# microsoft/GenerativeImage2Text

Hardware: NVIDIA H100
Metric: captions/sec (greedy, max_len=40) GIT_BASE batch64 (higher is better)
Workload: dtype bf16

## Files before the change

generativeimage2text_b200/_lib.py:

```python
import ctypes
import os

HERE = os.path.dirname(os.path.abspath(__file__))
LIB_PATH = os.path.join(HERE, 'libgitb200.so')
ABI_VERSION = 12

c_void_p, c_int, c_int64, c_float, c_char_p = ctypes.c_void_p, ctypes.c_int, ctypes.c_int64, ctypes.c_float, ctypes.c_char_p
c_ll = ctypes.c_longlong


class Config(ctypes.Structure):
    _fields_ = [(n, ctypes.c_int32) for n in (
        'image_size', 'patch', 'enc_width', 'enc_layers', 'enc_heads', 'dec_hidden', 'dec_layers', 'dec_heads',
        'dec_ffn', 'vocab', 'max_positions', 'num_frames_emb', 'sos_id', 'eos_id')]


class Search(ctypes.Structure):
    _fields_ = [('mode', ctypes.c_int32), ('max_steps', ctypes.c_int32), ('beam_size', ctypes.c_int32),
                ('per_node_beam', ctypes.c_int32), ('length_penalty', ctypes.c_float)]


class ImageDesc(ctypes.Structure):
    _fields_ = [('src_offset', ctypes.c_int64), ('src_h', ctypes.c_int32), ('src_w', ctypes.c_int32),
                ('resize_h', ctypes.c_int32), ('resize_w', ctypes.c_int32), ('crop_top', ctypes.c_int32),
                ('crop_left', ctypes.c_int32), ('out_h', ctypes.c_int32), ('out_w', ctypes.c_int32),
                ('dst_offset', ctypes.c_int64)]


# ... 33 lines not shown
    'gitb200_last_decode_ms': (c_int, [c_void_p, ctypes.POINTER(ctypes.c_float), ctypes.POINTER(ctypes.c_int32), ctypes.POINTER(ctypes.c_int32)]),
    'gitb200_set_row_prefixes': (c_int, [c_void_p, c_void_p, c_int, c_int, c_void_p]),
    'gitb200_set_trie': (c_int, [c_void_p, c_void_p, c_void_p, c_void_p, c_int, c_int]),
    'gitb200_set_sampling': (c_int, [c_void_p, c_void_p, c_int, c_int, c_float]),
    'gitb200_set_beam_sampling': (c_int, [c_void_p, c_void_p, c_int, c_int, c_float, c_int, c_float]),
    'gitb200_set_sequences_per_image': (c_int, [c_void_p, c_int]),
    'gitb200_launch_count': (c_int64, [c_void_p]),
    'gitb200_set_option': (c_int, [c_void_p, c_char_p, c_int64]),
    'gitb200_preproc_create': (c_int, [c_int, ctypes.POINTER(c_void_p)]),
    'gitb200_preproc_destroy': (None, [c_void_p]),
    'gitb200_preproc_last_error': (c_char_p, [c_void_p]),
    'gitb200_preproc_launch_count': (c_int64, [c_void_p]),
    'gitb200_preproc_set_option': (c_int, [c_void_p, c_char_p, c_int64]),
    'gitb200_preproc_run': (c_int, [c_void_p, c_void_p, c_int64, c_int, ctypes.POINTER(ImageDesc), c_int,
                                    ctypes.POINTER(c_float), ctypes.POINTER(c_float), c_void_p, c_int64, c_void_p]),
    'gitb200_preproc_coeffs': (c_int, [c_int, c_int, ctypes.POINTER(ctypes.c_int32), c_void_p, c_void_p, c_int]),
    'gitb200_debug_timeline': (c_int, [c_int, c_void_p, c_int]),
    'gitb200_debug_read': (c_ll, [c_void_p, c_char_p, c_void_p, c_ll]),
    'gitb200_op_gemm': (c_int, [c_void_p, c_void_p, c_void_p, c_void_p, c_void_p, c_int, c_int, c_int, c_int, c_int,
                                c_int, c_int, c_int, c_void_p]),
    'gitb200_op_layernorm': (c_int, [c_void_p, c_void_p, c_void_p, c_void_p, c_void_p, c_float, c_void_p, c_void_p,
                                     c_int, c_int, c_void_p]),
    'gitb200_op_gemm_ex': (c_int, [ctypes.POINTER(GemmDesc), ctypes.POINTER(c_int), c_void_p]),
    'gitb200_op_layernorm_ex': (c_int, [c_void_p, c_int, c_ll, c_void_p, c_void_p, c_void_p, c_void_p, c_float, c_void_p,
                                        c_void_p, c_int, c_int, c_int, c_void_p, c_int, c_int, c_int, c_void_p, c_int,
                                        c_void_p]),
    'gitb200_op_lse_combine': (c_int, [c_void_p, c_int, c_int, c_int, c_int, c_void_p, c_void_p, c_float, c_void_p,
                                       c_void_p, c_void_p, c_void_p, c_void_p]),
    'gitb200_op_attention': (c_int, [c_void_p, c_void_p, c_void_p, c_void_p, c_int, c_int, c_int, c_ll, c_ll, c_ll, c_ll,
                                     c_ll, c_ll, c_void_p]),
    'gitb200_op_attention_ex': (c_int, [c_void_p, c_void_p, c_void_p, c_void_p, c_int, c_int, c_int, c_ll, c_ll, c_ll,
                                        c_ll, c_ll, c_ll, ctypes.POINTER(ctypes.c_int32), c_int, c_void_p]),
    'gitb200_score': (c_int, [c_void_p, c_void_p, c_int, c_int, c_void_p, c_void_p, c_void_p, c_int, c_int, c_void_p,
                               c_void_p, c_void_p]),
    'gitb200_op_text_attention': (c_int, [c_void_p, c_void_p, c_void_p, c_void_p, c_void_p, c_void_p, c_int, c_int, c_int,
                                          c_int, ctypes.POINTER(ctypes.c_int32), ctypes.POINTER(ctypes.c_int32), c_int, c_int,
                                          c_void_p]),
    'gitb200_op_decode_attention': (c_int, [c_void_p, c_int, c_void_p, c_void_p, c_void_p, c_void_p, c_void_p, c_void_p,
                                            c_void_p, c_int, c_int, c_int, ctypes.POINTER(ctypes.c_int32), c_int, c_int,
                                            c_int, c_int, c_int, c_void_p]),
    'gitb200_op_beam_sample': (c_int, [c_void_p, c_int, c_int, c_void_p, c_void_p, c_float, c_int, c_float, c_void_p,
                                       c_void_p, c_void_p, c_void_p]),
}

_lib = None

# ... 30 lines not shown
```

generativeimage2text_b200/csrc/decode_mega.cuh:

```cuda
#pragma once
#include "ptx.cuh"
#include "rowops.cuh"

#include <type_traits>

namespace gitb200 {

constexpr int kMegaComputeWarps = 8;
constexpr int kMegaThreads = (kMegaComputeWarps + 1) * 32;
constexpr int kMegaSlots = 12;
constexpr int kMegaSlotBytes = 16384;
constexpr int kMegaTileBytes = 12288;
constexpr int kMegaKvRows = 64;
constexpr int kMegaKvSubRows = 16;
constexpr int kMegaMaxRows = 64;
constexpr int kMegaD = 768, kMegaF = 3072, kMegaH = 12;
constexpr int kMegaAttItems = 6;
constexpr int kMegaOutTiles = kMegaD / 8;
constexpr int kMegaQkvTiles = 3 * kMegaD / 8;
constexpr int kMegaFcTilesPerCta = 3;
constexpr int kMegaFcCtas = kMegaF / 8 / kMegaFcTilesPerCta;
constexpr int kMegaFc2Slices = kMegaF / kMegaD;
constexpr int kMegaMinCtas = kMegaFcCtas;
constexpr int kMegaAttState = 72;
constexpr unsigned int kMegaSpinLimit = 1u << 18;

struct MegaLayer {
  const uint8_t* wqkv;
  const uint8_t* wo;
  const uint8_t* w1;
  const uint8_t* w2;
  const float* bqkv; const float* bo; const float* b1; const float* b2;
  const float* lnag; const float* lnab; const float* lnog; const float* lnob;
  __nv_bfloat16* txt_k;
  __nv_bfloat16* txt_v;
};

struct MegaParams {
  MegaLayer layer[6];
  const uint8_t* lm;
  const float* lm_bias;
  const float* words;
  const float* positions;
  const float* lnemb_g; const float* lnemb_b;
  int M, T_alloc, n_layers;
  float* x;
  float* y;
  float* ypart;
// ... 73 lines not shown
      buf[2 * n] = t; buf[2 * n + 1] = static_cast<unsigned long long>(kid); ++n;
    }
  }
  __device__ __forceinline__ void end() {
    if (buf != nullptr) { mark(700002); if (n < 160u) { buf[2 * n] = globaltimer_ns(); buf[2 * n + 1] = 700003ull; ++n; } }
  }
};
#define MEGA_TL(kid) tlf.mark(kid)
#define MEGA_TL_DEP(a, error) if (((a).lo[5][7] ^ (a).hi[5][7] ^ (a).lo[0][0]) == 0x9E3779B9u) *(error) = kWaitTimelineProbe;
#else
struct MegaTl {
  __device__ __forceinline__ void begin() {}
  __device__ __forceinline__ void mark(int) {}
  __device__ __forceinline__ void end() {}
};
#define MEGA_TL(kid)
#define MEGA_TL_DEP(a, error)
#endif

__device__ __forceinline__ void bulk_load_1d(void* smem_dst, const void* gsrc, uint32_t bytes, uint64_t* bar) {
  asm volatile("cp.async.bulk.shared::cluster.global.mbarrier::complete_tx::bytes [%0], [%1], %2, [%3];"
               ::"r"(smem_u32(smem_dst)), "l"(gsrc), "r"(bytes), "r"(smem_u32(bar)) : "memory");
}
__device__ __forceinline__ bool mbar_wait_bounded(uint64_t* bar, uint32_t parity, const int* error) {
  for (unsigned int i = 0; i < kMegaSpinLimit; ++i) {
    if (mbar_try_wait(bar, parity)) return true;
    if ((i & 1023u) == 1023u && *reinterpret_cast<const volatile int*>(error) != 0) return false;
  }
  return false;
}

struct MegaRing {
  uint8_t* base;
  uint64_t* full;
  uint64_t* empty;
  uint32_t idx;
  int* error;
  volatile uint32_t* issued;
  __device__ __forceinline__ const uint8_t* acquire() {
    const uint32_t slot = idx % kMegaSlots;
    if (!mbar_wait_bounded(&full[slot], (idx / kMegaSlots) & 1, error)) *error = kWaitRingFull;
    return base + slot * kMegaSlotBytes;
  }
  __device__ __forceinline__ const uint8_t* acquire_ahead(uint32_t n) {
    const uint32_t i = idx + n, slot = i % kMegaSlots;
    if (!mbar_wait_bounded(&full[slot], (i / kMegaSlots) & 1, error)) *error = kWaitRingFull;
    return base + slot * kMegaSlotBytes;
  }
  __device__ __forceinline__ void release() {
    __syncwarp();
    if ((threadIdx.x & 31) == 0) mbar_arrive(&empty[idx % kMegaSlots]);
    ++idx;
  }
  __device__ __forceinline__ uint8_t* acquire_at(uint32_t i) {
// ... 643 lines not shown
```

generativeimage2text_b200/csrc/engine_api.inc:

```

extern "C" int gitb200_encode(gitb200_engine* h, const float* images_dev, int batch, int frames, float* feats_out_dev,
                              void* stream) {
  if (!h) return 1;
  const gitb200_engine::NextCall in = take_next_call(h, false);
  ImageBatch ib;
  TRY(image_batch(h, "encode", batch, frames, in.image_hw, &ib));
  if (!images_dev) return fail(h, "encode: null images");
  cudaSetDevice(h->device);
  return encode_impl(h, images_dev, ib, feats_out_dev, static_cast<cudaStream_t>(stream));
}

static int init_src_rows(gitb200_engine* h, cudaStream_t st) {
  const int n = h->cur_rows * h->T_alloc;
  init_src_row_kernel<<<(n + 255) / 256, 256, 0, st>>>(h->src_row[0].as<int>(), h->cur_rows, h->T_alloc);
  CKL(h, "init_src_row_kernel");
  init_src_row_kernel<<<(n + 255) / 256, 256, 0, st>>>(h->src_row[1].as<int>(), h->cur_rows, h->T_alloc);
  CKL(h, "init_src_row_kernel");
  h->cur_src = 0;
  return 0;
}

extern "C" int gitb200_prefill(gitb200_engine* h, int batch, int beam, float* vproj_out_dev, void* stream) {
  if (!h) return 1;
  cudaSetDevice(h->device);
// ... 158 lines not shown
  CKL(h, "greedy_select_kernel");
  return 0;
}

static int work_stream(gitb200_engine* h, cudaStream_t user, cudaStream_t* out) {
  if (user != nullptr && user != cudaStreamLegacy && user != cudaStreamPerThread) {
    *out = user;
    return 0;
  }
  if (h->own_stream == nullptr) {
    CK(cudaStreamCreateWithFlags(&h->own_stream, cudaStreamNonBlocking));
    CK(cudaEventCreateWithFlags(&h->own_event, cudaEventDisableTiming));
  }
  CK(cudaEventRecord(h->own_event, user));
  CK(cudaStreamWaitEvent(h->own_stream, h->own_event, 0));
  *out = h->own_stream;
  return 0;
}

static int generate_finish(gitb200_engine* h, int32_t* out_len_host) {
  if (!h->pending) return fail(h, "generate_finish: no generate call in flight");
  CK(cudaStreamSynchronize(h->pend_stream));
  h->pending = false;
  if (h->host_state[3].error != 0)
    return fail(h, "decode_mega_kernel: a bounded wait gave up (code %d: %s)", h->host_state[3].error,
                mega_wait_error_name(h->host_state[3].error));
  if (h->host_state[3].bad_draw != 0) {
    const int at = 0x7fffffff - h->host_state[3].bad_draw;
    return fail(h, "beam sampling: step %d, row %d has fewer than two tokens of non-zero probability to draw "
                "(torch.multinomial raises on it)", at / h->pend_rows, at % h->pend_rows);
  }
  if (out_len_host) {
    if (h->pend_beam) {
      *out_len_host = h->pend_max_steps;
    } else {
      *out_len_host = h->host_state[3].empty_caption ? -1 : h->host_state[3].final_len;
    }
  }
  return 0;
}

static int grow_text_cache(gitb200_engine* h, int new_T, SearchCtx* c, cudaStream_t st) {
  const int D = h->D, R = h->cur_rows, nl = h->cfg.dec_layers, old_T = h->T_alloc;
  if (new_T <= old_T) return 0;
  DevBuf nkv, nsrc[2];
  const size_t eb = h->kvb();
// ... 561 lines not shown
                d.row_offset, static_cast<long long>(d.batch_stride));
  GemmCall c;
  c.A = static_cast<const bf16*>(d.a); c.lda = d.lda; c.B = static_cast<const bf16*>(d.b); c.ldb = d.ldb;
  c.bn = d.bn;
  GemmParams& p = c.p;
  p.M = d.M; p.N = d.N; p.K = d.K; p.k_splits = d.k_splits;
  p.transposed = d.transposed ? 1 : 0; p.partial = d.k_splits > 1 ? 1 : 0; p.split_stride = d.split_stride;
  p.act = d.act; p.out_bf16 = d.out_bf16 ? 1 : 0; p.split3 = d.split3 ? 1 : 0;
  p.bias = d.bias; p.resid = d.resid; p.ld_resid = d.ld_resid;
  for (int s = 0; s < 3; ++s) p.out[s] = d.out[s];
  p.ldo = d.ldo; p.seg_n = d.seg_n;
  p.rows_per_batch = d.rows_per_batch; p.batch_stride = d.batch_stride; p.row_offset = d.rows_per_batch > 0 ? d.row_offset : 0;
  p.lse_target = d.lse_target; p.skip = d.skip;
  if (k_splits_out) *k_splits_out = effective_k_splits(d.K, d.k_splits);
  return launch_gemm(h, c, st);
}

extern "C" int gitb200_op_gemm_ex(const gitb200_gemm_desc* desc, int* k_splits_out, void* stream) {
  gitb200_engine* h = op_engine();
  if (!h) return fail(nullptr, "op_gemm_ex: no CUDA device");
  const int rc = desc ? op_gemm_ex_impl(h, *desc, k_splits_out, static_cast<cudaStream_t>(stream))
                      : fail(h, "op_gemm_ex: null descriptor");
  if (rc != 0) g_create_error = h->err;
  return rc;
}

static int op_layernorm_ex_impl(gitb200_engine* h, LnParams p, int D, int pre, cudaStream_t st) {
  if (!p.x || !p.gamma || !p.beta) return fail(h, "op_layernorm_ex: null input");
  if (p.rows < 1) return fail(h, "op_layernorm_ex: rows %d < 1", p.rows);
  if (p.n_partials < 1) return fail(h, "op_layernorm_ex: n_partials %d < 1", p.n_partials);
  if (p.n_partials > 1 && p.partial_stride < static_cast<long long>(p.rows) * D)
    return fail(h, "op_layernorm_ex: partial_stride smaller than one partial buffer");
  if (p.split3 && !p.out_bf16) return fail(h, "op_layernorm_ex: split3 is a bf16 output format");
  if (p.remap_F < 0 || (p.remap_F > 0 && (p.remap_B < 1 || p.remap_L < 1 || p.rows != p.remap_B * p.remap_F * p.remap_L)))
    return fail(h, "op_layernorm_ex: %d rows are not B=%d x F=%d x L=%d", p.rows, p.remap_B, p.remap_F, p.remap_L);
  if (p.temb && p.remap_F == 0) return fail(h, "op_layernorm_ex: a temporal embedding needs the frame remap");
  if (pre && D != 768) return fail(h, "op_layernorm_ex: the PRE instantiation exists for D = 768 only");
  return launch_ln(h, p, D, st, pre != 0);
}

extern "C" int gitb200_op_layernorm_ex(const float* x_dev, int n_partials, long long partial_stride, const float* bias_dev,
                                       const float* resid_dev, const float* gamma_dev, const float* beta_dev, float eps,
                                       float* out_f32_dev, void* out_bf16_dev, int rows, int D, int split3,
                                       const float* temb_dev, int remap_B, int remap_F, int remap_L,
                                       const int32_t* skip_flag_dev, int pre, void* stream) {
  gitb200_engine* h = op_engine();
// ... 292 lines not shown
```

generativeimage2text_b200/csrc/gemm.cuh:

```cuda
#pragma once
#include "ptx.cuh"

namespace gitb200 {

struct GemmParams {
  int M, N, K;
  int k_splits;
  int transposed;
  int partial;
  long long split_stride;
  int act;
  int out_bf16;
  const float* bias;
  const float* resid;
  long long ld_resid;
  void* out[3];
  long long ldo;
  long long batch_stride;
  int seg_n;
  int rows_per_batch;
  int row_offset;
  const int* skip;
  unsigned long long* dbg;
  int split3;
  int pdl;
  ChainSync chain;
  const int* lse_target;
};

constexpr int EPI_TRANSPOSED = 1, EPI_BF16 = 2, EPI_RESID = 4, EPI_PARTIAL = 8, EPI_ACT_SHIFT = 4, EPI_SPLIT3 = 64;
constexpr int EPI_LSE = 128;
constexpr int epi_code(bool transposed, bool bf16, bool resid, bool partial, int act) {
  return (transposed ? EPI_TRANSPOSED : 0) | (bf16 ? EPI_BF16 : 0) | (resid ? EPI_RESID : 0) | (partial ? EPI_PARTIAL : 0) |
         (act << EPI_ACT_SHIFT);
}

template <int ACT>
__device__ __forceinline__ float act_ct(float x) {
  return apply_act(x, ACT);
}

template <int BN>
struct GemmCfg {
  static constexpr int BM = 128;
  static constexpr int BK = 64;
  static constexpr int A_BYTES = BM * BK * 2;
  static constexpr int B_BYTES = BN * BK * 2;
  static constexpr int STAGE_BYTES = A_BYTES + B_BYTES;
  static constexpr int MMA_WGS = 2;
  static constexpr int THREADS = 128 * (1 + MMA_WGS);
// ... 176 lines not shown
  for (int it = 0; it < 8; ++it) {
    const int rr = it * 4 + rsub;
    const float4 v = *reinterpret_cast<const float4*>(stg + rr * 128 + ((c4 ^ (rr & 7)) << 4));
    const float x[4] = {v.x + b[0], v.y + b[1], v.z + b[2], v.w + b[3]};
    float cm = -INFINITY;
#pragma unroll
    for (int e = 0; e < 4; ++e) if (ok[e]) cm = fmaxf(cm, x[e]);
    const float nm = fmaxf(m[it], cm);
    if (nm == -INFINITY) continue;
    float acc = (m[it] == -INFINITY) ? 0.f : se[it] * __expf(m[it] - nm);
#pragma unroll
    for (int e = 0; e < 4; ++e) {
      if (ok[e]) {
        acc += __expf(x[e] - nm);
        sx[it] += x[e];
        if (tgt[it] == col0 + e) xt[it] = x[e];
      }
    }
    se[it] = acc;
    m[it] = nm;
  }
}

template <int BN, int EPI>
__global__ void __launch_bounds__(GemmCfg<BN>::THREADS, 1)
gemm_bf16_wgmma(const __grid_constant__ CUtensorMap tmA, const __grid_constant__ CUtensorMap tmB,
                const GemmParams p) {
  using C = GemmCfg<BN>;
  constexpr bool kTransposed = (EPI & EPI_TRANSPOSED) != 0;
  constexpr bool kLse = (EPI & EPI_LSE) != 0;
  static_assert(!kLse || EPI == EPI_LSE, "the statistics epilogue takes no other option");
  if (p.pdl) griddep_launch_early();
  if (p.pdl) tl_mark(100000 + 1000 + static_cast<int>(gridDim.x));
  if ((!p.pdl || p.chain.counters != nullptr) && p.skip != nullptr && *p.skip != 0) return;
  extern __shared__ __align__(1024) uint8_t smem_raw[];
  uint8_t* smem = smem_raw + ((1024u - (smem_u32(smem_raw) & 1023u)) & 1023u);
  uint8_t* sA = smem;
  uint8_t* sB = smem + C::STAGES * C::A_BYTES;
  uint8_t* sStage = smem + C::STAGES * C::STAGE_BYTES;
  uint64_t* full = reinterpret_cast<uint64_t*>(sStage + C::STAGING_BYTES);
  uint64_t* empty = full + C::STAGES;

  const int wg = threadIdx.x >> 7;
  const int warp = (threadIdx.x >> 5) & 3;
  const int lane = threadIdx.x & 31;

  if (threadIdx.x == 0) {
    tma_prefetch_desc(&tmA);
    tma_prefetch_desc(&tmB);
    for (int s = 0; s < C::STAGES; ++s) {
      mbar_init(&full[s], 1);
      mbar_init(&empty[s], C::MMA_WGS);
    }
    mbar_fence_init();
  }
  __syncthreads();

  const int m_tiles = (p.M + C::BM - 1) / C::BM;
  const int n_tiles = (p.N + BN - 1) / BN;
  const int kb_total = (p.K + C::BK - 1) / C::BK;
  const int kb_per = (kb_total + p.k_splits - 1) / p.k_splits;
  const int mn_tiles = m_tiles * n_tiles;
  const int num_tiles = mn_tiles * p.k_splits;

  const bool chained = p.chain.counters != nullptr;
  int npre = 0;
  if (kTransposed && p.pdl && static_cast<int>(blockIdx.x) < num_tiles) {
    const int split = static_cast<int>(blockIdx.x) / mn_tiles;
    const int kb0 = split * kb_per;
    npre = min(C::STAGES, min(kb_total, kb0 + kb_per) - kb0);
    if (threadIdx.x == 0) {
      const int m_blk = (static_cast<int>(blockIdx.x) - split * mn_tiles) / n_tiles;
      for (int i = 0; i < npre; ++i) {
        mbar_arrive_expect_tx(&full[i], C::STAGE_BYTES);
        tma_load_2d(sA + i * C::A_BYTES, &tmA, &full[i], (kb0 + i) * C::BK, m_blk * C::BM);
      }
    }
  }
  if (chained) chain_wait(p.chain);
  else if (p.pdl) griddep_wait();
  if (p.pdl) tl_mark(1000 + static_cast<int>(gridDim.x));

  if (wg == 0) {
    setmaxnreg_dec<C::PRODUCER_REGS>();
    if (threadIdx.x == 0) {
      int stage = 0;
      uint32_t phase = 0;
      for (int tile = blockIdx.x; tile < num_tiles; tile += gridDim.x) {
        const int split = tile / mn_tiles;
        const int rem = tile - split * mn_tiles;
        const int m_blk = rem / n_tiles;
        const int n_blk = rem - m_blk * n_tiles;
        const int kb0 = split * kb_per;
        const int kb1 = min(kb_total, kb0 + kb_per);
        for (int kb = kb0; kb < kb1; ++kb) {
          if (npre > 0) {
            --npre;
            tma_load_2d(sB + stage * C::B_BYTES, &tmB, &full[stage], kb * C::BK, n_blk * BN);
          } else {
            mbar_wait(&empty[stage], phase ^ 1);
            mbar_arrive_expect_tx(&full[stage], C::STAGE_BYTES);
            tma_load_2d(sA + stage * C::A_BYTES, &tmA, &full[stage], kb * C::BK, m_blk * C::BM);
            tma_load_2d(sB + stage * C::B_BYTES, &tmB, &full[stage], kb * C::BK, n_blk * BN);
          }
          if (++stage == C::STAGES) {
            stage = 0;
            phase ^= 1;
          }
        }
      }
    }
  } else {
    setmaxnreg_inc<C::MMA_REGS>();
    const int mw = wg - 1;
    const bool store_ok = !(p.pdl && !chained && p.skip != nullptr && *p.skip != 0);
    uint8_t* stg_wg = sStage + mw * C::WG_STAGING_BYTES;
    uint8_t* stg = stg_wg + warp * (32 * 128);
    const int rsub = lane >> 3;
    float acc[BN / 2];
    int stage = 0;
    uint32_t phase = 0;
    for (int tile = blockIdx.x; tile < num_tiles; tile += gridDim.x) {
      const int split = tile / mn_tiles;
      const int rem = tile - split * mn_tiles;
      const int m_blk = rem / n_tiles;
      const int n_blk = rem - m_blk * n_tiles;
      const int kb0 = split * kb_per;
      const int kb1 = min(kb_total, kb0 + kb_per);
      int prev = -1;
      for (int kb = kb0; kb < kb1; ++kb) {
        mbar_wait(&full[stage], phase);
        if (p.pdl && tile == static_cast<int>(blockIdx.x) && kb == kb0 && threadIdx.x == 128) tl_mark_one(300000 + 1000 + static_cast<int>(gridDim.x));
        const uint32_t a_base = smem_u32(sA + stage * C::A_BYTES + mw * (64 * 128));
        const uint32_t b_base = smem_u32(sB + stage * C::B_BYTES);
        wgmma_fence();
#pragma unroll
        for (int k = 0; k < C::BK / 16; ++k)
          Wgmma<BN>::mma(acc, wgmma_desc_sw128(a_base + k * 32), wgmma_desc_sw128(b_base + k * 32), (kb > kb0 || k > 0) ? 1u : 0u);
        wgmma_commit();
        if (prev >= 0) {
          wgmma_wait<1>();
          if ((threadIdx.x & 127) == 0) mbar_arrive(&empty[prev]);
        }
        prev = stage;
        if (++stage == C::STAGES) {
          stage = 0;
          phase ^= 1;
        }
      }
      wgmma_wait<0>();
      if ((threadIdx.x & 127) == 0) mbar_arrive(&empty[prev]);
      if (p.pdl && tile == static_cast<int>(blockIdx.x) && threadIdx.x == 128) tl_mark_one(400000 + 1000 + static_cast<int>(gridDim.x));

      const int row0 = m_blk * C::BM + mw * 64 + (warp & 1) * 32;
      long long ooff[8];
      uint32_t okmask = 0;
      if (!kTransposed && !kLse) okmask = epi_row_offsets(p, row0, rsub, store_ok, ooff);
      float lm[8], lse_s[8], lsx[8], lxt[8];
      int ltg[8];
      if constexpr (kLse) {
#pragma unroll
        for (int it = 0; it < 8; ++it) {
          const int row = row0 + it * 4 + rsub;
          ltg[it] = row < p.M ? p.lse_target[row] : -1;
          lm[it] = -INFINITY; lse_s[it] = 0.f; lsx[it] = 0.f; lxt[it] = 0.f;
        }
      }
#pragma unroll
      for (int cc = 0; cc < BN / 64; ++cc) {
        if (n_blk * BN + cc * 64 >= p.N) break;
#pragma unroll
        for (int j8 = 0; j8 < 8; ++j8) {
#pragma unroll
          for (int hh = 0; hh < 2; ++hh) {
// ... 25 lines not shown
#pragma unroll
        for (int it = 0; it < 8; ++it) {
#pragma unroll
          for (int o = 1; o < 8; o <<= 1) {
            const float m_o = __shfl_xor_sync(0xffffffffu, lm[it], o);
            const float s_o = __shfl_xor_sync(0xffffffffu, lse_s[it], o);
            const float nm = fmaxf(lm[it], m_o);
            const float sa = (lm[it] == -INFINITY) ? 0.f : lse_s[it] * __expf(lm[it] - nm);
            const float sb = (m_o == -INFINITY) ? 0.f : s_o * __expf(m_o - nm);
            lse_s[it] = sa + sb;
            lm[it] = nm;
            lsx[it] += __shfl_xor_sync(0xffffffffu, lsx[it], o);
            lxt[it] += __shfl_xor_sync(0xffffffffu, lxt[it], o);
          }
          const int row = row0 + it * 4 + rsub;
          if ((lane & 7) == 0 && row < p.M)
            reinterpret_cast<float4*>(p.out[0])[static_cast<long long>(row) * p.ldo + 2 * n_blk + (warp >> 1)] =
                make_float4(lm[it], lse_s[it], lsx[it], lxt[it]);
        }
      }
    }
  }

  __syncthreads();
  if (p.pdl) tl_mark(200000 + 1000 + static_cast<int>(gridDim.x));
  if (chained && threadIdx.x == 0) chain_signal_thread0(p.chain);
}

}
```

generativeimage2text_b200/csrc/gitb200.cu:

```cuda
#include <cuda.h>
#include <cuda_bf16.h>
#include <cuda_runtime.h>

#include <algorithm>
#include <atomic>
#include <cmath>
#include <cstdarg>
#include <cstdio>
#include <cstring>
#include <map>
#include <mutex>
#include <set>
#include <string>
#include <utility>
#include <vector>

#include "../../include/gitb200.h"
#include "attention.cuh"
#include "constrained.cuh"
#include "decode_mega.cuh"
#include "gemm.cuh"
#include "preproc.cuh"
#include "ptx.cuh"
#include "rowops.cuh"
#include "search.cuh"

using namespace gitb200;
typedef __nv_bfloat16 bf16;

#define GITB200_ABI_VERSION 12

static thread_local std::string g_create_error;

struct DevBuf {
  static inline std::atomic<unsigned long long> moves{0};
  void* p = nullptr;
  size_t cap = 0;
  bool owned = true;
  cudaError_t ensure(size_t bytes) {
    if (bytes <= cap) return cudaSuccess;
    if (!owned) return cudaErrorInvalidValue;
    if (p) cudaFree(p);
    p = nullptr;
    cap = 0;
    ++moves;
    cudaError_t e = cudaMalloc(&p, bytes);
    if (e == cudaSuccess) cap = bytes;
    return e;
  }
  void release() {
    if (p) ++moves;
    if (p && owned) cudaFree(p);
    p = nullptr;
// ... 88 lines not shown
  DevBuf img_kv, txt_kv, src_row[2];
  size_t txt_kv_eb = 0;
  DevBuf xd_t, hd_t, qkv_t, ctx_t, t_t, u_t, logits;
  DevBuf y_t, qb_t, mega_bar;
  DevBuf state, next_token, logprob_sum, tokens_i64, stage_img, stage_tok, stage_lp, prefix_dev;
  DevBuf beam_ws;
  BeamState beam_s{};
  int beam_B = 0, beam_max_steps = 0;
  int beam_cand = 0;
  DevBuf sc_kv, sc_tgt, sc_part, sc_loss, sc_valid, sc_index;
  DevBuf sel_ws;
  DevBuf chain;
  DecAttnGeom attn_geom{};
  int cur_B = 0, cur_frames = 0, cur_M = 0, cur_beam = 1, T_alloc = 0, cur_rows = 0, cur_src = 0;
  int cur_seqs = 1;

  EncodeTiledFn encode_tiled = nullptr;
  std::map<TmapKey, CUtensorMap> tmaps;

  struct StepGraph { cudaGraphExec_t exec = nullptr; int64_t launches = 0; unsigned long long last_use = 0; };
  std::map<std::string, StepGraph> step_graphs;
  unsigned long long step_graph_clock = 0;
  int last_gemm_grid = 0;
  cudaStream_t own_stream = nullptr;
  cudaEvent_t own_event = nullptr;
  StepState* host_state = nullptr;
  bool pending = false;
  int pend_max_steps = 0;
  int pend_rows = 0;
  bool pend_beam = false;
  cudaStream_t pend_stream = nullptr;
  cudaEvent_t chunk_ev[2] = {nullptr, nullptr};
  cudaEvent_t dec_ev[2] = {nullptr, nullptr};
  int dec_steps = 0;
  bool dec_mega = false;
  DevBuf trie_begin, trie_token, trie_child, trie_cursor;
  int trie_nodes = 0;
  struct NextCall {
    std::vector<int> image_hw;
    const long long* prefix_tok = nullptr;
    const int32_t* prefix_lens = nullptr;
    int prefix_rows = 0, prefix_stride = 0;
    const float* uniforms = nullptr;
    int sample_steps = 0, sample_rows = 0;
    float temperature = 1.0f;
    const float* beam_uniforms = nullptr;
// ... 99 lines not shown

static int set_dyn_smem(gitb200_engine* h, const void* kernel, size_t smem) {
  static std::mutex mu;
  static std::map<std::pair<const void*, int>, size_t> done;
  std::lock_guard<std::mutex> lock(mu);
  size_t& have = done[{kernel, h->device}];
  if (have < smem) {
    CK(cudaFuncSetAttribute(kernel, cudaFuncAttributeMaxDynamicSharedMemorySize, static_cast<int>(smem)));
    have = smem;
  }
  return 0;
}

struct GemmCall {
  const bf16* A = nullptr;
  long long lda = 0;
  const bf16* B = nullptr;
  long long ldb = 0;
  GemmParams p{};
  int bn = 0;
};

template <int BN, int EPI>
static int launch_gemm_inst(gitb200_engine* h, const GemmCall& c, cudaStream_t st) {
  using C = GemmCfg<BN>;
  TRY(set_dyn_smem(h, reinterpret_cast<const void*>(gemm_bf16_wgmma<BN, EPI>), C::SMEM_BYTES));
  CUtensorMap ta, tb;
  TRY(get_tmap(h, c.A, c.p.M, c.p.K, c.lda, 128, &ta));
  TRY(get_tmap(h, c.B, c.p.N, c.p.K, c.ldb, BN, &tb));
  const int m_tiles = (c.p.M + 127) / 128;
  const int n_tiles = (c.p.N + BN - 1) / BN;
  const int tiles = m_tiles * n_tiles * c.p.k_splits;
  const int grid = tiles < h->num_sms ? tiles : h->num_sms;
  h->last_gemm_grid = grid;
  CK(launch_k(c.p.pdl != 0, gemm_bf16_wgmma<BN, EPI>, dim3(grid), dim3(C::THREADS), C::SMEM_BYTES, st, ta, tb, c.p));
  CKL(h, "gemm_bf16_wgmma");
  return 0;
}

template <int BN>
static int launch_gemm_bn(gitb200_engine* h, const GemmCall& c, cudaStream_t st) {
  const GemmParams& p = c.p;
  if constexpr (BN == 256) {
    if (p.lse_target != nullptr) return launch_gemm_inst<BN, EPI_LSE>(h, c, st);
  }
  if (p.lse_target != nullptr) return fail(h, "gemm: the LM-head statistics epilogue runs with 256-column tiles only");
  const int code = epi_code(p.transposed != 0, p.out_bf16 != 0, p.resid != nullptr, p.partial != 0, p.act) | (p.split3 ? EPI_SPLIT3 : 0);
  if constexpr (BN == 256) {
    switch (code) {
      case epi_code(false, true, false, false, ACT_QUICKGELU_EXACT) | EPI_SPLIT3: return launch_gemm_inst<BN, epi_code(false, true, false, false, ACT_QUICKGELU_EXACT) | EPI_SPLIT3>(h, c, st);
      case epi_code(false, true, false, false, ACT_GELU_ERF) | EPI_SPLIT3: return launch_gemm_inst<BN, epi_code(false, true, false, false, ACT_GELU_ERF) | EPI_SPLIT3>(h, c, st);
      default: break;
    }
  }
// ... 359 lines not shown
  logprob_sum[r] = 0.f;
}
__global__ void advance_prefix_kernel(StepState* st, long long* next_token, const long long* prefix, int idx, int rows,
                                      unsigned int* chain) {
  const int r = blockIdx.x * blockDim.x + threadIdx.x;
  if (r < rows) next_token[r] = prefix[idx];
  if (r == 0) st->pos = st->pos + 1;
  if (r < 64) chain[r] = 0;
}

extern "C" int gitb200_abi_version(void) { return GITB200_ABI_VERSION; }

extern "C" const char* gitb200_last_error(const gitb200_engine* h) { return h ? h->err.c_str() : g_create_error.c_str(); }

extern "C" int64_t gitb200_launch_count(const gitb200_engine* h) { return h ? h->launches : 0; }

extern "C" int gitb200_set_option(gitb200_engine* h, const char* name, int64_t value) {
  if (!h || !name) return 1;
  drop_step_graphs(h);
  if (strcmp(name, "use_graph") == 0) { h->use_graph = value != 0; return 0; }
  if (strcmp(name, "use_pdl") == 0) { h->use_pdl = value != 0; return 0; }
  if (strcmp(name, "use_mega") == 0) { h->use_mega = value != 0; return 0; }
  if (strcmp(name, "debug_layers") == 0) { h->debug_layers = static_cast<int>(value); return 0; }
  if (strcmp(name, "parity") == 0) {
    if (h->weights_from != nullptr) return fail(h, "parity: this engine borrows its weights; switch the owning engine");
    if (h->parity != (value != 0)) { h->parity = value != 0; h->finalized = false; h->seen.clear(); h->tmaps.clear(); }
    return 0;
  }
  return fail(h, "unknown option %s", name);
}

static int check_image_size(gitb200_engine* h, const char* what, int b, int height, int width) {
  const int p = h->cfg.patch;
  const long long tokens = static_cast<long long>(height / p) * (width / p) + 1;
  if (b < 0) {
    if (height < p || width < p) return fail(h, "%s: %dx%d is smaller than one %dx%d patch", what, height, width, p, p);
    if (tokens > 16384) return fail(h, "%s: %dx%d gives %lld tokens per image (limit 16384)", what, height, width, tokens);
    return 0;
  }
  if (height < p || width < p) return fail(h, "%s: image %d is %dx%d, smaller than one %dx%d patch", what, b, height, width, p, p);
  if (tokens > 16384) return fail(h, "%s: image %d (%dx%d) gives %lld tokens (limit 16384)", what, b, height, width, tokens);
  return 0;
}

extern "C" int gitb200_set_input_size(gitb200_engine* h, int height, int width) {
  if (!h) return 1;
// ... 654 lines not shown
```

generativeimage2text_b200/csrc/ptx.cuh:

```cuda
#pragma once
#include <cuda.h>
#include <cuda_bf16.h>
#include <cuda_runtime.h>
#include <stdint.h>

namespace gitb200 {

__device__ __forceinline__ uint32_t smem_u32(const void* p) {
  return static_cast<uint32_t>(__cvta_generic_to_shared(p));
}
__device__ __forceinline__ int lane_id() { return threadIdx.x & 31; }
__device__ __forceinline__ unsigned long long globaltimer_ns() {
  unsigned long long t;
  asm volatile("mov.u64 %0, %%globaltimer;" : "=l"(t));
  return t;
}

#ifdef GITB200_TIMELINE
__device__ unsigned long long* g_tl_buf = nullptr;
__device__ unsigned int g_tl_count = 0;
constexpr unsigned int kTimelineMax = 8192;
__device__ __forceinline__ void tl_mark_one(int kid) {
  if (g_tl_buf != nullptr && blockIdx.x == 0 && blockIdx.y == 0 && blockIdx.z == 0) {
    const unsigned int i = atomicAdd(&g_tl_count, 1u);
// ... 68 lines not shown
  asm volatile("mbarrier.arrive.expect_tx.shared::cta.b64 _, [%0], %1;" ::"r"(smem_u32(bar)), "r"(bytes)
               : "memory");
}
__device__ __forceinline__ void mbar_arrive(uint64_t* bar) {
  asm volatile("mbarrier.arrive.shared::cta.b64 _, [%0];" ::"r"(smem_u32(bar)) : "memory");
}
__device__ __forceinline__ bool mbar_try_wait(uint64_t* bar, uint32_t parity) {
  uint32_t ok;
  asm volatile(
      "{\n"
      ".reg .pred p;\n"
      "mbarrier.try_wait.parity.shared::cta.b64 p, [%1], %2;\n"
      "selp.u32 %0, 1, 0, p;\n"
      "}\n"
      : "=r"(ok)
      : "r"(smem_u32(bar)), "r"(parity)
      : "memory");
  return ok != 0;
}
__device__ __forceinline__ void mbar_wait(uint64_t* bar, uint32_t parity) {
  while (!mbar_try_wait(bar, parity)) {
  }
}

__device__ __forceinline__ void tma_prefetch_desc(const CUtensorMap* m) {
  asm volatile("prefetch.tensormap [%0];" ::"l"(reinterpret_cast<uint64_t>(m)) : "memory");
}
__device__ __forceinline__ void tma_load_2d(void* smem_dst, const CUtensorMap* m, uint64_t* bar, int c_inner,
                                            int c_outer) {
  asm volatile(
      "cp.async.bulk.tensor.2d.shared::cluster.global.mbarrier::complete_tx::bytes [%0], [%1, {%3, %4}], [%2];"
      ::"r"(smem_u32(smem_dst)), "l"(reinterpret_cast<uint64_t>(m)), "r"(smem_u32(bar)), "r"(c_inner),
      "r"(c_outer)
      : "memory");
}

__device__ __forceinline__ void wgmma_fence() { asm volatile("wgmma.fence.sync.aligned;" ::: "memory"); }
__device__ __forceinline__ void wgmma_commit() { asm volatile("wgmma.commit_group.sync.aligned;" ::: "memory"); }
template <int N>
__device__ __forceinline__ void wgmma_wait() {
  asm volatile("wgmma.wait_group.sync.aligned %0;" ::"n"(N) : "memory");
}
template <int R>
__device__ __forceinline__ void setmaxnreg_dec() { asm volatile("setmaxnreg.dec.sync.aligned.u32 %0;" ::"n"(R)); }
template <int R>
__device__ __forceinline__ void setmaxnreg_inc() { asm volatile("setmaxnreg.inc.sync.aligned.u32 %0;" ::"n"(R)); }

__device__ __forceinline__ uint64_t wgmma_desc_sw128(uint32_t smem_addr) {
  uint64_t d = 0;
  d |= static_cast<uint64_t>((smem_addr & 0x3FFFF) >> 4);
  d |= static_cast<uint64_t>(1) << 16;
  d |= static_cast<uint64_t>(1024 >> 4) << 32;
  d |= static_cast<uint64_t>(1) << 62;
  return d;
}

// ... 159 lines not shown
```

include/gitb200.h:

```cpp
#ifndef GITB200_H_
#define GITB200_H_

#include <stdint.h>

#ifdef __cplusplus
extern "C" {
#endif

typedef struct gitb200_engine gitb200_engine;

typedef struct gitb200_config {
  int32_t image_size;
  int32_t patch;
  int32_t enc_width;
  int32_t enc_layers;
  int32_t enc_heads;
  int32_t dec_hidden;
  int32_t dec_layers;
  int32_t dec_heads;
  int32_t dec_ffn;
  int32_t vocab;
  int32_t max_positions;
  int32_t num_frames_emb;
  int32_t sos_id;
// ... 71 lines not shown
int64_t gitb200_launch_count(const gitb200_engine* h);
int gitb200_set_option(gitb200_engine* h, const char* name, int64_t value);

int gitb200_op_gemm(const void* a_dev, const void* w_dev, const float* bias_dev, const float* resid_dev,
                    void* out_dev, int M, int N, int K, int act, int out_bf16, int transposed, int k_splits,
                    int bn, void* stream);
int gitb200_op_layernorm(const float* x_dev, const float* bias_dev, const float* resid_dev, const float* gamma_dev,
                         const float* beta_dev, float eps, float* out_f32_dev, void* out_bf16_dev, int rows, int D,
                         void* stream);
typedef struct gitb200_gemm_desc {
  const void* a;
  const void* b;
  const float* bias;
  const float* resid;
  void* out[3];
  const int32_t* lse_target;
  const int32_t* skip;
  int64_t lda, ldb, ld_resid, ldo, batch_stride, split_stride;
  int32_t M, N, K;
  int32_t act, out_bf16, split3, transposed, k_splits, bn;
  int32_t seg_n, rows_per_batch, row_offset;
} gitb200_gemm_desc;
int gitb200_op_gemm_ex(const gitb200_gemm_desc* desc, int* k_splits_out, void* stream);
int gitb200_op_layernorm_ex(const float* x_dev, int n_partials, long long partial_stride, const float* bias_dev,
                            const float* resid_dev, const float* gamma_dev, const float* beta_dev, float eps,
                            float* out_f32_dev, void* out_bf16_dev, int rows, int D, int split3, const float* temb_dev,
                            int remap_B, int remap_F, int remap_L, const int32_t* skip_flag_dev, int pre, void* stream);
int gitb200_op_lse_combine(const void* parts_dev, int n_parts, int rows, int T, int V, const int32_t* targets_dev,
                           const int64_t* need_predict_dev, float eps, float* logprob_dev, float* row_loss_dev,
                           int32_t* row_valid_dev, float* loss_dev, void* stream);
int gitb200_op_attention(const void* q_dev, const void* k_dev, const void* v_dev, void* out_dev, int B, int S, int H,
                         long long q_row_stride, long long kv_row_stride, long long q_batch_stride,
                         long long kv_batch_stride, long long out_row_stride, long long out_batch_stride,
                         void* stream);
int gitb200_op_attention_ex(const void* q_dev, const void* k_dev, const void* v_dev, void* out_dev, int B, int S, int H,
                            long long q_row_stride, long long kv_row_stride, long long q_batch_stride,
                            long long kv_batch_stride, long long out_row_stride, long long out_batch_stride,
                            const int32_t* seq_lens_host, int fp32, void* stream);
int gitb200_op_decode_attention(const float* qkv_dev, int n_partials, const float* bqkv_dev, const void* img_k_dev,
                                const void* img_v_dev, void* txt_k_dev, void* txt_v_dev, const int32_t* src_row_dev,
                                void* ctx_dev, int B, int beam, int M, const int32_t* img_lens_host, int T_alloc, int pos,
                                int D, int fp32, int grid, void* stream);

int gitb200_op_beam_sample(const float* logits_dev, int rows, int V, const float* beam_scores_dev, const float* uniforms_dev,
                           float temperature, int top_k, float top_p, float* cand_val_out_dev, int32_t* cand_idx_out_dev,
                           int32_t* kept_out_dev, void* stream);
// ... 33 lines not shown
```

Before: 3013.

## Add 2-CTA cluster GEMM variant with TMA multicast of shared B tiles

Adds a paired form of the wgmma GEMM where two CTAs in a cluster compute adjacent M tiles and each loads half of the shared B tile, multicasting it to both CTAs. Empty-slot barriers are released across the cluster. A heuristic picks the paired form when the estimated bytes loaded per round drop, and only for non-PDL, non-chained plain-epilogue GEMMs. The aim is to cut global and L2 traffic for the weight operand, at the cost of cluster synchronisation, bounded spin waits that report errors, and an extra device-to-host error check at generate_finish.

```diff
diff --git a/generativeimage2text_b200/_lib.py b/generativeimage2text_b200/_lib.py
--- a/generativeimage2text_b200/_lib.py
+++ b/generativeimage2text_b200/_lib.py
@@ -3,7 +3,7 @@
 
 HERE = os.path.dirname(os.path.abspath(__file__))
 LIB_PATH = os.path.join(HERE, 'libgitb200.so')
-ABI_VERSION = 12
+ABI_VERSION = 13
 
 c_void_p, c_int, c_int64, c_float, c_char_p = ctypes.c_void_p, ctypes.c_int, ctypes.c_int64, ctypes.c_float, ctypes.c_char_p
 c_ll = ctypes.c_longlong
@@ -83,6 +83,7 @@
     'gitb200_op_layernorm': (c_int, [c_void_p, c_void_p, c_void_p, c_void_p, c_void_p, c_float, c_void_p, c_void_p,
                                      c_int, c_int, c_void_p]),
     'gitb200_op_gemm_ex': (c_int, [ctypes.POINTER(GemmDesc), ctypes.POINTER(c_int), c_void_p]),
+    'gitb200_op_gemm_pair': (c_int, [c_int]),
     'gitb200_op_layernorm_ex': (c_int, [c_void_p, c_int, c_ll, c_void_p, c_void_p, c_void_p, c_void_p, c_float, c_void_p,
                                         c_void_p, c_int, c_int, c_int, c_void_p, c_int, c_int, c_int, c_void_p, c_int,
                                         c_void_p]),
diff --git a/generativeimage2text_b200/csrc/decode_mega.cuh b/generativeimage2text_b200/csrc/decode_mega.cuh
--- a/generativeimage2text_b200/csrc/decode_mega.cuh
+++ b/generativeimage2text_b200/csrc/decode_mega.cuh
@@ -23,7 +23,7 @@
 constexpr int kMegaFc2Slices = kMegaF / kMegaD;
 constexpr int kMegaMinCtas = kMegaFcCtas;
 constexpr int kMegaAttState = 72;
-constexpr unsigned int kMegaSpinLimit = 1u << 18;
+constexpr unsigned int kMegaSpinLimit = kSpinLimit;
 
 struct MegaLayer {
   const uint8_t* wqkv;
@@ -143,14 +143,6 @@
   asm volatile("cp.async.bulk.shared::cluster.global.mbarrier::complete_tx::bytes [%0], [%1], %2, [%3];"
                ::"r"(smem_u32(smem_dst)), "l"(gsrc), "r"(bytes), "r"(smem_u32(bar)) : "memory");
 }
-__device__ __forceinline__ bool mbar_wait_bounded(uint64_t* bar, uint32_t parity, const int* error) {
-  for (unsigned int i = 0; i < kMegaSpinLimit; ++i) {
-    if (mbar_try_wait(bar, parity)) return true;
-    if ((i & 1023u) == 1023u && *reinterpret_cast<const volatile int*>(error) != 0) return false;
-  }
-  return false;
-}
-
 struct MegaRing {
   uint8_t* base;
   uint64_t* full;
diff --git a/generativeimage2text_b200/csrc/engine_api.inc b/generativeimage2text_b200/csrc/engine_api.inc
--- a/generativeimage2text_b200/csrc/engine_api.inc
+++ b/generativeimage2text_b200/csrc/engine_api.inc
@@ -204,6 +204,7 @@
   if (!h->pending) return fail(h, "generate_finish: no generate call in flight");
   CK(cudaStreamSynchronize(h->pend_stream));
   h->pending = false;
+  TRY(check_gemm_waits(h, h->pend_stream));
   if (h->host_state[3].error != 0)
     return fail(h, "decode_mega_kernel: a bounded wait gave up (code %d: %s)", h->host_state[3].error,
                 mega_wait_error_name(h->host_state[3].error));
@@ -811,6 +812,18 @@
   const int rc = desc ? op_gemm_ex_impl(h, *desc, k_splits_out, static_cast<cudaStream_t>(stream))
                       : fail(h, "op_gemm_ex: null descriptor");
   if (rc != 0) g_create_error = h->err;
+  return rc;
+}
+
+extern "C" int gitb200_op_gemm_pair(int mode) {
+  gitb200_engine* h = op_engine();
+  if (!h) return fail(nullptr, "op_gemm_pair: no CUDA device");
+  int rc = 0;
+  if (mode < -1 || mode > 1) rc = fail(h, "op_gemm_pair: mode %d is not -1, 0 or 1", mode);
+  else if (cudaDeviceSynchronize() != cudaSuccess) rc = fail(h, "op_gemm_pair: device synchronise failed");
+  else rc = check_gemm_waits(h, nullptr);
+  if (rc == 0) h->gemm_pair = mode;
+  else g_create_error = h->err;
   return rc;
 }
 
diff --git a/generativeimage2text_b200/csrc/gemm.cuh b/generativeimage2text_b200/csrc/gemm.cuh
--- a/generativeimage2text_b200/csrc/gemm.cuh
+++ b/generativeimage2text_b200/csrc/gemm.cuh
@@ -26,6 +26,12 @@
   int pdl;
   ChainSync chain;
   const int* lse_target;
+  int* error;
+};
+
+enum GemmWaitError : int {
+  kGemmWaitFull = 1,
+  kGemmWaitEmpty = 2,
 };
 
 constexpr int EPI_TRANSPOSED = 1, EPI_BF16 = 2, EPI_RESID = 4, EPI_PARTIAL = 8, EPI_ACT_SHIFT = 4, EPI_SPLIT3 = 64;
@@ -248,7 +254,11 @@
   }
 }
 
-template <int BN, int EPI>
+__host__ __device__ constexpr bool gemm_pairable(int epi) {
+  return (epi & (EPI_TRANSPOSED | EPI_PARTIAL | EPI_SPLIT3 | EPI_LSE)) == 0;
+}
+
+template <int BN, int EPI, bool kPair = false>
 __global__ void __launch_bounds__(GemmCfg<BN>::THREADS, 1)
 gemm_bf16_wgmma(const __grid_constant__ CUtensorMap tmA, const __grid_constant__ CUtensorMap tmB,
                 const GemmParams p) {
@@ -256,6 +266,8 @@
   constexpr bool kTransposed = (EPI & EPI_TRANSPOSED) != 0;
   constexpr bool kLse = (EPI & EPI_LSE) != 0;
   static_assert(!kLse || EPI == EPI_LSE, "the statistics epilogue takes no other option");
+  static_assert(!kPair || gemm_pairable(EPI), "the paired form runs the plain normal shape only");
+  constexpr int kHalfB = C::B_BYTES / 2;
   if (p.pdl) griddep_launch_early();
   if (p.pdl) tl_mark(100000 + 1000 + static_cast<int>(gridDim.x));
   if ((!p.pdl || p.chain.counters != nullptr) && p.skip != nullptr && *p.skip != 0) return;
@@ -276,18 +288,23 @@
     tma_prefetch_desc(&tmB);
     for (int s = 0; s < C::STAGES; ++s) {
       mbar_init(&full[s], 1);
-      mbar_init(&empty[s], C::MMA_WGS);
+      mbar_init(&empty[s], C::MMA_WGS * (kPair ? 2 : 1));
     }
     mbar_fence_init();
   }
   __syncthreads();
+  if constexpr (kPair) cluster_sync();
+  const uint32_t rank = kPair ? cluster_ctarank() : 0u;
 
   const int m_tiles = (p.M + C::BM - 1) / C::BM;
   const int n_tiles = (p.N + BN - 1) / BN;
   const int kb_total = (p.K + C::BK - 1) / C::BK;
   const int kb_per = (kb_total + p.k_splits - 1) / p.k_splits;
-  const int mn_tiles = m_tiles * n_tiles;
+  const int m_units = kPair ? (m_tiles + 1) / 2 : m_tiles;
+  const int mn_tiles = m_units * n_tiles;
   const int num_tiles = mn_tiles * p.k_splits;
+  const int first_tile = kPair ? static_cast<int>(blockIdx.x) / 2 : static_cast<int>(blockIdx.x);
+  const int tile_step = kPair ? static_cast<int>(gridDim.x) / 2 : static_cast<int>(gridDim.x);
 
   const bool chained = p.chain.counters != nullptr;
   int npre = 0;
@@ -312,15 +329,22 @@
     if (threadIdx.x == 0) {
       int stage = 0;
       uint32_t phase = 0;
-      for (int tile = blockIdx.x; tile < num_tiles; tile += gridDim.x) {
+      for (int tile = first_tile; tile < num_tiles; tile += tile_step) {
         const int split = tile / mn_tiles;
         const int rem = tile - split * mn_tiles;
-        const int m_blk = rem / n_tiles;
-        const int n_blk = rem - m_blk * n_tiles;
+        const int m_unit = rem / n_tiles;
+        const int n_blk = rem - m_unit * n_tiles;
+        const int m_blk = kPair ? 2 * m_unit + static_cast<int>(rank) : m_unit;
         const int kb0 = split * kb_per;
         const int kb1 = min(kb_total, kb0 + kb_per);
         for (int kb = kb0; kb < kb1; ++kb) {
-          if (npre > 0) {
+          if constexpr (kPair) {
+            if (!mbar_wait_bounded(&empty[stage], phase ^ 1, p.error)) *p.error = kGemmWaitEmpty;
+            mbar_arrive_expect_tx(&full[stage], C::STAGE_BYTES);
+            tma_load_2d(sA + stage * C::A_BYTES, &tmA, &full[stage], kb * C::BK, m_blk * C::BM);
+            tma_load_2d_multicast(sB + stage * C::B_BYTES + rank * kHalfB, &tmB, &full[stage], kb * C::BK,
+                                  n_blk * BN + static_cast<int>(rank) * (BN / 2), 0x3);
+          } else if (npre > 0) {
             --npre;
             tma_load_2d(sB + stage * C::B_BYTES, &tmB, &full[stage], kb * C::BK, n_blk * BN);
           } else {
@@ -346,16 +370,31 @@
     float acc[BN / 2];
     int stage = 0;
     uint32_t phase = 0;
-    for (int tile = blockIdx.x; tile < num_tiles; tile += gridDim.x) {
+    auto release = [&](int slot) {
+      if ((threadIdx.x & 127) == 0) {
+        if constexpr (kPair) {
+          mbar_arrive_cluster(&empty[slot], 0);
+          mbar_arrive_cluster(&empty[slot], 1);
+        } else {
+          mbar_arrive(&empty[slot]);
+        }
+      }
+    };
+    for (int tile = first_tile; tile < num_tiles; tile += tile_step) {
       const int split = tile / mn_tiles;
       const int rem = tile - split * mn_tiles;
-      const int m_blk = rem / n_tiles;
-      const int n_blk = rem - m_blk * n_tiles;
+      const int m_unit = rem / n_tiles;
+      const int n_blk = rem - m_unit * n_tiles;
+      const int m_blk = kPair ? 2 * m_unit + static_cast<int>(rank) : m_unit;
       const int kb0 = split * kb_per;
       const int kb1 = min(kb_total, kb0 + kb_per);
       int prev = -1;
       for (int kb = kb0; kb < kb1; ++kb) {
-        mbar_wait(&full[stage], phase);
+        if constexpr (kPair) {
+          if (!mbar_wait_bounded(&full[stage], phase, p.error)) *p.error = kGemmWaitFull;
+        } else {
+          mbar_wait(&full[stage], phase);
+        }
         if (p.pdl && tile == static_cast<int>(blockIdx.x) && kb == kb0 && threadIdx.x == 128) tl_mark_one(300000 + 1000 + static_cast<int>(gridDim.x));
         const uint32_t a_base = smem_u32(sA + stage * C::A_BYTES + mw * (64 * 128));
         const uint32_t b_base = smem_u32(sB + stage * C::B_BYTES);
@@ -366,7 +405,7 @@
         wgmma_commit();
         if (prev >= 0) {
           wgmma_wait<1>();
-          if ((threadIdx.x & 127) == 0) mbar_arrive(&empty[prev]);
+          release(prev);
         }
         prev = stage;
         if (++stage == C::STAGES) {
@@ -375,7 +414,7 @@
         }
       }
       wgmma_wait<0>();
-      if ((threadIdx.x & 127) == 0) mbar_arrive(&empty[prev]);
+      release(prev);
       if (p.pdl && tile == static_cast<int>(blockIdx.x) && threadIdx.x == 128) tl_mark_one(400000 + 1000 + static_cast<int>(gridDim.x));
 
       const int row0 = m_blk * C::BM + mw * 64 + (warp & 1) * 32;
@@ -447,7 +486,8 @@
     }
   }
 
-  __syncthreads();
+  if constexpr (kPair) cluster_sync();
+  else __syncthreads();
   if (p.pdl) tl_mark(200000 + 1000 + static_cast<int>(gridDim.x));
   if (chained && threadIdx.x == 0) chain_signal_thread0(p.chain);
 }
diff --git a/generativeimage2text_b200/csrc/gitb200.cu b/generativeimage2text_b200/csrc/gitb200.cu
--- a/generativeimage2text_b200/csrc/gitb200.cu
+++ b/generativeimage2text_b200/csrc/gitb200.cu
@@ -28,7 +28,7 @@
 using namespace gitb200;
 typedef __nv_bfloat16 bf16;
 
-#define GITB200_ABI_VERSION 12
+#define GITB200_ABI_VERSION 13
 
 static thread_local std::string g_create_error;
 
@@ -163,6 +163,8 @@
   std::map<std::string, StepGraph> step_graphs;
   unsigned long long step_graph_clock = 0;
   int last_gemm_grid = 0;
+  int gemm_pair = -1;
+  DevBuf gemm_err;
   cudaStream_t own_stream = nullptr;
   cudaEvent_t own_event = nullptr;
   StepState* host_state = nullptr;
@@ -308,14 +310,100 @@
 };
 
 template <int BN, int EPI>
+static int pair_clusters(gitb200_engine* h, int* out) {
+  using C = GemmCfg<BN>;
+  static std::mutex mu;
+  static std::map<int, int> done;
+  const auto kern = gemm_bf16_wgmma<BN, EPI, true>;
+  TRY(set_dyn_smem(h, reinterpret_cast<const void*>(kern), C::SMEM_BYTES));
+  std::lock_guard<std::mutex> lock(mu);
+  auto it = done.find(h->device);
+  if (it == done.end()) {
+    cudaLaunchConfig_t cfg{};
+    cfg.gridDim = dim3(2 * h->num_sms);
+    cfg.blockDim = dim3(C::THREADS);
+    cfg.dynamicSmemBytes = C::SMEM_BYTES;
+    cudaLaunchAttribute attr[1];
+    attr[0].id = cudaLaunchAttributeClusterDimension;
+    attr[0].val.clusterDim.x = 2; attr[0].val.clusterDim.y = 1; attr[0].val.clusterDim.z = 1;
+    cfg.attrs = attr;
+    cfg.numAttrs = 1;
+    int n = 0;
+    CK(cudaOccupancyMaxActiveClusters(&n, kern, &cfg));
+    it = done.emplace(h->device, n).first;
+  }
+  *out = it->second;
+  return 0;
+}
+
+static bool gemm_pair_wins(int m_tiles, int n_tiles, int a_bytes, int b_bytes, int sms, int clusters) {
+  const long long rounds = (static_cast<long long>(m_tiles) * n_tiles + sms - 1) / sms;
+  const long long pair_rounds = (static_cast<long long>((m_tiles + 1) / 2) * n_tiles + clusters - 1) / clusters;
+  return pair_rounds * (a_bytes + b_bytes / 2) < rounds * (a_bytes + b_bytes);
+}
+
+static int gemm_error_word(gitb200_engine* h, int** out) {
+  if (h->gemm_err.p == nullptr) {
+    CK(h->gemm_err.ensure(sizeof(int)));
+    CK(cudaMemset(h->gemm_err.p, 0, sizeof(int)));
+  }
+  *out = h->gemm_err.as<int>();
+  return 0;
+}
+static int check_gemm_waits(gitb200_engine* h, cudaStream_t st) {
+  if (h->gemm_err.p == nullptr) return 0;
+  int code = 0;
+  CK(cudaMemcpyAsync(&code, h->gemm_err.p, sizeof(int), cudaMemcpyDeviceToHost, st));
+  CK(cudaStreamSynchronize(st));
+  if (code == 0) return 0;
+  CK(cudaMemset(h->gemm_err.p, 0, sizeof(int)));
+  return fail(h, "gemm_bf16_wgmma (paired form): a bounded wait gave up (code %d: %s)", code,
+              code == kGemmWaitFull ? "the peer's half of a B tile never landed" :
+              code == kGemmWaitEmpty ? "the peer never freed a slot" : "unknown code");
+}
+
+template <int BN, int EPI>
+static int launch_gemm_pair(gitb200_engine* h, const GemmCall& c, int clusters, cudaStream_t st) {
+  using C = GemmCfg<BN>;
+  CUtensorMap ta, tb;
+  TRY(get_tmap(h, c.A, c.p.M, c.p.K, c.lda, 128, &ta));
+  TRY(get_tmap(h, c.B, c.p.N, c.p.K, c.ldb, BN / 2, &tb));
+  GemmParams p = c.p;
+  TRY(gemm_error_word(h, &p.error));
+  cudaLaunchConfig_t cfg{};
+  cfg.gridDim = dim3(2 * clusters);
+  cfg.blockDim = dim3(C::THREADS);
+  cfg.dynamicSmemBytes = C::SMEM_BYTES;
+  cfg.stream = st;
+  cudaLaunchAttribute attr[1];
+  attr[0].id = cudaLaunchAttributeClusterDimension;
+  attr[0].val.clusterDim.x = 2; attr[0].val.clusterDim.y = 1; attr[0].val.clusterDim.z = 1;
+  cfg.attrs = attr;
+  cfg.numAttrs = 1;
+  h->last_gemm_grid = 2 * clusters;
+  CK(cudaLaunchKernelEx(&cfg, gemm_bf16_wgmma<BN, EPI, true>, ta, tb, p));
+  CKL(h, "gemm_bf16_wgmma (paired)");
+  return 0;
+}
+
+template <int BN, int EPI>
 static int launch_gemm_inst(gitb200_engine* h, const GemmCall& c, cudaStream_t st) {
   using C = GemmCfg<BN>;
+  const int m_tiles = (c.p.M + 127) / 128;
+  const int n_tiles = (c.p.N + BN - 1) / BN;
+  if constexpr (gemm_pairable(EPI)) {
+    if (h->gemm_pair != 0 && !c.p.pdl && c.p.chain.counters == nullptr) {
+      int clusters = 0;
+      TRY((pair_clusters<BN, EPI>(h, &clusters)));
+      if (clusters > 0 &&
+          (h->gemm_pair == 1 || gemm_pair_wins(m_tiles, n_tiles, C::A_BYTES, C::B_BYTES, h->num_sms, clusters)))
+        return launch_gemm_pair<BN, EPI>(h, c, std::min(clusters, (m_tiles + 1) / 2 * n_tiles), st);
+    }
+  }
   TRY(set_dyn_smem(h, reinterpret_cast<const void*>(gemm_bf16_wgmma<BN, EPI>), C::SMEM_BYTES));
   CUtensorMap ta, tb;
   TRY(get_tmap(h, c.A, c.p.M, c.p.K, c.lda, 128, &ta));
   TRY(get_tmap(h, c.B, c.p.N, c.p.K, c.ldb, BN, &tb));
-  const int m_tiles = (c.p.M + 127) / 128;
-  const int n_tiles = (c.p.N + BN - 1) / BN;
   const int tiles = m_tiles * n_tiles * c.p.k_splits;
   const int grid = tiles < h->num_sms ? tiles : h->num_sms;
   h->last_gemm_grid = grid;
@@ -721,6 +809,11 @@
   if (strcmp(name, "use_pdl") == 0) { h->use_pdl = value != 0; return 0; }
   if (strcmp(name, "use_mega") == 0) { h->use_mega = value != 0; return 0; }
   if (strcmp(name, "debug_layers") == 0) { h->debug_layers = static_cast<int>(value); return 0; }
+  if (strcmp(name, "gemm_pair") == 0) {
+    if (value < -1 || value > 1) return fail(h, "gemm_pair: %lld is not -1, 0 or 1", static_cast<long long>(value));
+    h->gemm_pair = static_cast<int>(value);
+    return 0;
+  }
   if (strcmp(name, "parity") == 0) {
     if (h->weights_from != nullptr) return fail(h, "parity: this engine borrows its weights; switch the owning engine");
     if (h->parity != (value != 0)) { h->parity = value != 0; h->finalized = false; h->seen.clear(); h->tmaps.clear(); }
diff --git a/generativeimage2text_b200/csrc/ptx.cuh b/generativeimage2text_b200/csrc/ptx.cuh
--- a/generativeimage2text_b200/csrc/ptx.cuh
+++ b/generativeimage2text_b200/csrc/ptx.cuh
@@ -114,6 +114,32 @@
   while (!mbar_try_wait(bar, parity)) {
   }
 }
+constexpr unsigned int kSpinLimit = 1u << 18;
+__device__ __forceinline__ bool mbar_wait_bounded(uint64_t* bar, uint32_t parity, const int* error) {
+  for (unsigned int i = 0; i < kSpinLimit; ++i) {
+    if (mbar_try_wait(bar, parity)) return true;
+    if ((i & 1023u) == 1023u && *reinterpret_cast<const volatile int*>(error) != 0) return false;
+  }
+  return false;
+}
+
+__device__ __forceinline__ uint32_t cluster_ctarank() {
+  uint32_t r;
+  asm volatile("mov.u32 %0, %%cluster_ctarank;" : "=r"(r));
+  return r;
+}
+__device__ __forceinline__ void cluster_sync() {
+  asm volatile("barrier.cluster.arrive.release.aligned;\nbarrier.cluster.wait.acquire.aligned;" ::: "memory");
+}
+__device__ __forceinline__ void mbar_arrive_cluster(uint64_t* bar, uint32_t cta) {
+  asm volatile(
+      "{\n"
+      ".reg .b32 remote;\n"
+      "mapa.shared::cluster.u32 remote, %0, %1;\n"
+      "mbarrier.arrive.release.cluster.shared::cluster.b64 _, [remote];\n"
+      "}\n"
+      ::"r"(smem_u32(bar)), "r"(cta) : "memory");
+}
 
 __device__ __forceinline__ void tma_prefetch_desc(const CUtensorMap* m) {
   asm volatile("prefetch.tensormap [%0];" ::"l"(reinterpret_cast<uint64_t>(m)) : "memory");
@@ -124,6 +150,15 @@
       "cp.async.bulk.tensor.2d.shared::cluster.global.mbarrier::complete_tx::bytes [%0], [%1, {%3, %4}], [%2];"
       ::"r"(smem_u32(smem_dst)), "l"(reinterpret_cast<uint64_t>(m)), "r"(smem_u32(bar)), "r"(c_inner),
       "r"(c_outer)
+      : "memory");
+}
+__device__ __forceinline__ void tma_load_2d_multicast(void* smem_dst, const CUtensorMap* m, uint64_t* bar, int c_inner,
+                                                      int c_outer, uint16_t cta_mask) {
+  asm volatile(
+      "cp.async.bulk.tensor.2d.shared::cluster.global.mbarrier::complete_tx::bytes.multicast::cluster"
+      " [%0], [%1, {%3, %4}], [%2], %5;"
+      ::"r"(smem_u32(smem_dst)), "l"(reinterpret_cast<uint64_t>(m)), "r"(smem_u32(bar)), "r"(c_inner), "r"(c_outer),
+        "h"(cta_mask)
       : "memory");
 }
 
diff --git a/include/gitb200.h b/include/gitb200.h
--- a/include/gitb200.h
+++ b/include/gitb200.h
@@ -117,6 +117,7 @@
   int32_t seg_n, rows_per_batch, row_offset;
 } gitb200_gemm_desc;
 int gitb200_op_gemm_ex(const gitb200_gemm_desc* desc, int* k_splits_out, void* stream);
+int gitb200_op_gemm_pair(int mode);
 int gitb200_op_layernorm_ex(const float* x_dev, int n_partials, long long partial_stride, const float* bias_dev,
                             const float* resid_dev, const float* gamma_dev, const float* beta_dev, float eps,
                             float* out_f32_dev, void* out_bf16_dev, int rows, int D, int split3, const float* temb_dev,
```

Result: slower. 2241 (median of 6 runs) (-25.6%).
